# blackfeather-wang/AdaFocus

Measured on AMD Instinct MI355X. Metric: clips/sec (T=16, patch=96^2, ResNet-50 local), higher is better.
Workload: dtype f32; 1 GPU; ActivityNet AdaFocus hot path: gather + ResNet-50 local CNN + GRU classifier, T=16, P=96, B=64 clips/GPU (1024 patches/GPU/step), random-init weights seed 1007; global_batch=64, frames=16, patch=96, parallelism=dp1, streams=3

## Files before the change

adafocus_amd/csrc/adaf_internal.h:

```cpp
#pragma once
#include <hip/hip_runtime.h>
#include <stdint.h>
#include <stddef.h>
#include <string>

#include "../../include/adafocus.h"
#include <type_traits>

struct adaf_handle {
    int device = 0;
    int cus = 256;
    float* zeros = nullptr;
    unsigned* scan_timeouts = nullptr;
    int conv_pos_major = 1;
    int gru_persistent = 1;
    hipEvent_t scan_done[4] = {nullptr, nullptr, nullptr, nullptr};
    bool scan_used[4] = {false, false, false, false};
    int scan_next = 0;
    int scan_resident = 0;
    int scan_slots = 1;
    int bptt_resident = 0;
    std::string err;
};

// ... 78 lines not shown
    }
};

struct AdafOptions {
    int conv_pool = 1;
    int mb_strip = 1;
    int mbv2_chunk = 512;
    int latency_rows = 1536;
    int latency_linear_rows = 128;
    unsigned effnet_plan = 511u;
    unsigned effnet_fused_blocks = 0xffffffffu;
    int effnet_chunk = 1024;
    int stem_rows = 1;
    int split_stage1_f32 = 1;
    int split_lean = 1;
    int tsm_lean = 1;
    int gru_graph_persistent = 0;
    int gru_scan_slices = 2;
};
AdafOptions& adaf_options();

__device__ __forceinline__ _Float16 adaf_f16_of(float v) {
#if defined(__HIP_DEVICE_COMPILE__)
    asm("" : "+v"(v));
#endif
    return (_Float16)v;
}

struct ConvArgs {
    const float* x;
// ... 8 lines not shown
    int ldx, ldo, ldr;
    int act;
    int tsm_T, tsm_fold, tsm_hw;
    const float* zeros;
    int vec_epi;
    int in16, out16, res16;
    int pm_allow;
    int split_n;
    float* out_b;
    int ldo_b, act_b;
    int pm_images, pm_groups;
    int tiles_n;
    int nblocks;
    int pool_hw, pool_rows, pool_ld;
    float* pool_out;
};

int adaf_fail(adaf_handle* h, int code, const char* fmt, ...);
int adaf_hip_fail(adaf_handle* h, hipError_t e, const char* what);
bool adaf_aligned16(const void* p);
enum AdafWsOrder { ADAF_WS_SIZE_FIRST, ADAF_WS_ALIGN_FIRST };
int adaf_check_ws(adaf_handle* h, const char* who, const void* ws, size_t ws_bytes, size_t need, AdafWsOrder order);
int adaf_conv_out(int in, int k, int stride, int pad);
int adaf_make_conv_args(adaf_handle* h, const adaf_conv_params* p, const float* x, const float* w, const float* scale,
                        const float* bias, const float* res, float* out, ConvArgs* a);
int adaf_set_conv_dtypes(adaf_handle* h, bool in16, bool out16, ConvArgs* a);

struct MbFuseArgs {
    const float* x;
    int n, H, W, cin;
// ... 83 lines not shown
                                           float* logits, float* last, int classes, bool cooperative, unsigned* timeouts, hipStream_t s);

int adaf_gru_bptt_blocks_per_cu();
bool adaf_gru_bptt_persistent_ok(int batch, int hidden, int resident_blocks);
hipError_t adaf_launch_gru_bptt(const float* dy, const float* gi, const float* gh, const float* bhh, const float* hs, const float* whh,
                                float* dgi, float* dgh, float* carry, unsigned* bar, unsigned* timeouts, int batch, int steps, int hidden,
                                bool persistent, bool cooperative, hipStream_t s);
void adaf_launch_gemm_strided(const float* A, long long a_m, long long a_k, const float* B, long long b_k, long long b_n, float* C, int ldc,
                              const float* mul, int ldm, int M, int N, int K, hipStream_t s);
size_t adaf_colsum_partial_floats(int cols);
void adaf_launch_colsum(const float* x, int rows, int cols, int ld, float* part, float* out, hipStream_t s);
void adaf_launch_rows_scale(const float* x, const float* mask, float* out, int rows, int width, int steps, bool shift, hipStream_t s);

int adaf_launch_conv_gemm(const ConvArgs& a, int tile, int cus, hipStream_t s);
int adaf_pick_conv_tile(int M, int N, int K, int cus);
int adaf_launch_conv_lat(const ConvArgs& a, hipStream_t s);
int adaf_launch_conv_pool(ConvArgs a, int hw, float* pool_out, int pool_ld, hipStream_t s);
int adaf_launch_conv_pool16(ConvArgs a, int hw, float* pool_out, int pool_ld, hipStream_t s);
int adaf_launch_conv_pool16_rounded(ConvArgs a, int hw, float* pool_out, int pool_ld, hipStream_t s);
bool adaf_conv_tile_exists(int tile);
void adaf_launch_conv_naive(const ConvArgs& a, hipStream_t s);
bool adaf_fused_tail_shift_ok(const ConvArgs& c2, int n3, int ldr, int tsm_T1, int tsm_fold1);
int adaf_launch_fused_tail(const ConvArgs& c2, const float* w3, const float* s3, const float* b3, const float* res, int ldr,
                           float* out, int n3, const float* w1n, const float* s1n, const float* b1n, float* out1, int n1,
                           hipStream_t s, int tsm_T1 = 0, int tsm_fold1 = 0);

hipError_t adaf_launch_crop(const float* frames, int nf, int C, int H, int W, const float* act, int fpa, int P,
                            float* out, int layout, int32_t* coords, hipStream_t s);

hipError_t adaf_launch_crop_resize(const float* frames, int in4, int nf, int C, int H, int W, const float* act, const int32_t* sizes,
// ... 44 lines not shown
```

adafocus_amd/csrc/api.hip:

```cpp
#include <cstdarg>
#include <cstdio>
#include <cstring>

#include "adaf_internal.h"

int adaf_fail(adaf_handle* h, int code, const char* fmt, ...) {
    char buf[512];
    va_list ap;
    va_start(ap, fmt);
    vsnprintf(buf, sizeof(buf), fmt, ap);
    va_end(ap);
    if (h) h->err = buf;
    return code;
}

int adaf_hip_fail(adaf_handle* h, hipError_t e, const char* what) {
    return adaf_fail(h, ADAF_E_LAUNCH, "%s: %s", what, hipGetErrorString(e));
}

bool adaf_aligned16(const void* p) { return (reinterpret_cast<uintptr_t>(p) & 15) == 0; }
int adaf_check_ws(adaf_handle* h, const char* who, const void* ws, size_t ws_bytes, size_t need, AdafWsOrder order) {
    const bool small = ws_bytes < need, skew = !adaf_aligned16(ws);
    if (small && (order == ADAF_WS_SIZE_FIRST || !skew)) return adaf_fail(h, ADAF_E_NOMEM, "%s: workspace %zu < %zu bytes", who, ws_bytes, need);
    return skew ? adaf_fail(h, ADAF_E_LAYOUT, "%s: the workspace must be 16-byte aligned", who) : ADAF_OK;
// ... 15 lines not shown
    if (oh <= 0 || ow <= 0) return adaf_fail(h, ADAF_E_BADARG, "conv: empty output");
    const long long M = (long long)p->n * oh * ow;
    if (M > 0x7fffffffLL || (long long)p->n * p->h * p->w > 0x7fffffffLL) return adaf_fail(h, ADAF_E_BADARG, "conv: too many pixels");
    int fold = 0;
    if (p->tsm_segments > 0) {
        if (p->kh != 1 || p->kw != 1 || p->stride != 1 || p->pad != 0)
            return adaf_fail(h, ADAF_E_BADARG, "conv: fused temporal shift needs a 1x1 stride-1 conv");
        if (p->tsm_div <= 0 || p->n % p->tsm_segments) return adaf_fail(h, ADAF_E_BADARG, "conv: n %% tsm_segments != 0");
        fold = p->cin / p->tsm_div;
        if (fold % 4) return adaf_fail(h, ADAF_E_LAYOUT, "conv: temporal-shift fold=%d must be a multiple of 4", fold);
    }
    a->wsp = nullptr;
    a->in16 = a->out16 = a->res16 = 0;
    a->pm_allow = h->conv_pos_major; a->pm_images = a->pm_groups = 0;
    a->split_n = 0; a->out_b = nullptr; a->ldo_b = 0; a->act_b = 0;
    a->x = x; a->w = w; a->scale = scale; a->bias = bias; a->res = res; a->out = out;
    a->M = (int)M; a->N = p->cout; a->K = p->kh * p->kw * p->cin;
    a->cin = p->cin; a->H = p->h; a->W = p->w; a->OH = oh; a->OW = ow; a->KH = p->kh; a->KW = p->kw;
    a->stride = p->stride; a->pad = p->pad; a->ldx = ldx; a->ldo = ldo; a->ldr = ldr; a->act = p->act;
    a->tsm_T = p->tsm_segments > 0 ? p->tsm_segments : 0; a->tsm_fold = fold; a->tsm_hw = p->h * p->w;
    a->tiles_n = 0; a->nblocks = 0;
    a->zeros = h->zeros;
    a->vec_epi = (p->cout % 4 == 0 && ldo % 4 == 0 && ldr % 4 == 0 && adaf_aligned16(out) && (!res || adaf_aligned16(res)) &&
                  (!scale || adaf_aligned16(scale)) && (!bias || adaf_aligned16(bias))) ? 1 : 0;
    return ADAF_OK;
}

int adaf_set_conv_dtypes(adaf_handle* h, bool in16, bool out16, ConvArgs* a) {
    a->in16 = in16; a->out16 = out16; a->res16 = a->res != nullptr;
    if (in16 && (a->cin % 8 || a->ldx % 8)) return adaf_fail(h, ADAF_E_LAYOUT, "conv_f16: fp16 operands need cin %% 8 == 0 (16-byte chunks)");
    if (in16 && a->tsm_T > 0 && a->tsm_fold % 8)
        return adaf_fail(h, ADAF_E_LAYOUT, "conv_f16: temporal-shift fold=%d must be a multiple of 8 with fp16 operands (whole 16-byte chunks)", a->tsm_fold);
    if (!in16 && a->res) return adaf_fail(h, ADAF_E_BADARG, "conv_f16: a residual needs fp16 operands");
    return ADAF_OK;
}

AdafOptions& adaf_options() {
    static AdafOptions o;
    return o;
}

namespace {
struct OptKey { const char* name; double lo, hi; };
const OptKey kOptKeys[] = {{"conv_pool", 0, 1}, {"mb_strip", 0, 1}, {"mbv2_chunk", 1, 1 << 20}, {"latency_rows", 0, 1 << 30}, {"latency_linear_rows", 0, 1 << 30},
                           {"effnet_plan", 0, 511}, {"effnet_chunk", 1, 1 << 20}, {"gru_scan_slices", 1, 2}, {"effnet_fused_blocks", 0, 4294967295.0},
                           {"stem_rows", 0, 2}, {"split_stage1_f32", 0, 1}, {"gru_graph_persistent", 0, 1}, {"split_lean", 0, 1}, {"tsm_lean", 0, 1}};
int find_opt(const char* key) {
    if (!key) return -1;
    for (size_t i = 0; i < sizeof(kOptKeys) / sizeof(kOptKeys[0]); ++i)
        if (!strcmp(kOptKeys[i].name, key)) return (int)i;
    return -1;
}
}

extern "C" {

int adaf_version(void) { return ADAF_VERSION; }

int adaf_create(int device, adaf_handle** out) {
    if (!out) return ADAF_E_BADARG;
    *out = nullptr;
// ... 50 lines not shown
    AdafOptions& o = adaf_options();
    switch (k) {
        case 0: o.conv_pool = (int)value; break;
        case 1: o.mb_strip = (int)value; break;
        case 2: o.mbv2_chunk = (int)value; break;
        case 3: o.latency_rows = (int)value; break;
        case 4: o.latency_linear_rows = (int)value; break;
        case 5: o.effnet_plan = (unsigned)value; break;
        case 6: o.effnet_chunk = (int)value; break;
        case 7: o.gru_scan_slices = (int)value; break;
        case 8: o.effnet_fused_blocks = (unsigned)value; break;
        case 9: o.stem_rows = (int)value; break;
        case 10: o.split_stage1_f32 = (int)value; break;
        case 11: o.gru_graph_persistent = (int)value; break;
        case 12: o.split_lean = (int)value; break;
        default: o.tsm_lean = (int)value; break;
    }
    return ADAF_OK;
}

double adaf_get_global_option(const char* key) {
    const AdafOptions& o = adaf_options();
    switch (find_opt(key)) {
        case 0: return o.conv_pool;
        case 1: return o.mb_strip;
        case 2: return o.mbv2_chunk;
        case 3: return o.latency_rows;
        case 4: return o.latency_linear_rows;
        case 5: return o.effnet_plan;
        case 6: return o.effnet_chunk;
        case 7: return o.gru_scan_slices;
        case 8: return o.effnet_fused_blocks;
        case 9: return o.stem_rows;
        case 10: return o.split_stage1_f32;
        case 11: return o.gru_graph_persistent;
        case 12: return o.split_lean;
        case 13: return o.tsm_lean;
        default: return __builtin_nan("");
    }
}

int adaf_set_gru_persistent(adaf_handle* h, int on) {
    if (!h) return ADAF_E_BADARG;
    if (on < 0 || on > 2) return adaf_fail(h, ADAF_E_BADARG, "set_gru_persistent: mode %d (0 off, 1 on, 2 on + cooperative launch)", on);
    h->gru_persistent = on;
    return ADAF_OK;
}

int adaf_gru_scan_timeouts(adaf_handle* h, unsigned* count_out) {
    if (!h || !count_out) return ADAF_E_BADARG;
    int cur = 0;
    (void)hipGetDevice(&cur);
// ... 528 lines not shown
```

adafocus_amd/csrc/conv_gemm.hip:

```cpp
#include <cstdlib>
#include <type_traits>
#include <utility>

#include "adaf_internal.h"

typedef float f32x16 __attribute__((ext_vector_type(16)));
typedef float f32x4 __attribute__((ext_vector_type(4)));
typedef float f32x2 __attribute__((ext_vector_type(2)));
typedef unsigned u32x4 __attribute__((ext_vector_type(4)));
typedef __bf16 bf16x8 __attribute__((ext_vector_type(8)));
typedef _Float16 f16x8 __attribute__((ext_vector_type(8)));
typedef _Float16 f16x4 __attribute__((ext_vector_type(4)));

#ifndef CG_ABL
#define CG_ABL 0
#endif

namespace {

typedef __bf16 bf16x2 __attribute__((ext_vector_type(2)));
__device__ __forceinline__ void split3(const f32x4 v0, const f32x4 v1, u32x4& H, u32x4& M, u32x4& L) {
    const float x[8] = {v0.x, v0.y, v0.z, v0.w, v1.x, v1.y, v1.z, v1.w};
    unsigned h[4], m[4], l[4];
#pragma unroll
// ... 440 lines not shown
        }
        if (FLAGS & 1) __builtin_amdgcn_s_setprio(0);
        __builtin_amdgcn_sched_barrier(0);
        if (more) lstore((kt + 1) & 1);
        __syncthreads();
    }

    conv_epilogue<TM, TN, ET>(a, smem, acc, m0, n0, wm, wn, lane, wave);
}


template <int BM, int BN, int WGM, int WGN, bool DENSE, int PIPE, bool SPECIAL, int EMU, bool BSP = false, int DT = 0, bool PM = false,
          bool LEAN = false, bool POOL = false>
__global__ __launch_bounds__(64 * WGM * WGN, (BM == 128 && BN == 128 && WGM * WGN == 4) ? 2 : 1)
void conv_gemm_glds_kernel(const ConvArgs a) {
    static_assert(!POOL || (DENSE && !SPECIAL && ((LEAN && DT == 0) || (!LEAN && (DT == 4 || DT == 6)))),
                  "pooled epilogue: the lean dense fp32 kernel, or the dense fp16-operand kernel with fp32 features (DT 6: fp16 residual, rounded values)");
    static_assert(!PM || (!DENSE && (EMU == 0 || BSP) && PIPE == 1), "position-major tiles: k x k filters on the fp32 pipe, or split tiles with pre-split weights");
    static_assert(!LEAN || ((DENSE || PM) && PIPE == 1 && ((EMU == 0 && !BSP) || (EMU != 0 && BSP)) &&
                            (!SPECIAL || (DENSE && EMU == 0 && DT == 0 && !POOL))),
                  "lean K loop: plain fp32-pipe launches, split tiles with pre-split weights, or (LEAN + SPECIAL) the fp32 pipe's temporally shifted conv1");
    constexpr bool LTSM = LEAN && SPECIAL;
    constexpr int NW = WGM * WGN;
    constexpr int TM = BM / WGM / 32, TN = BN / WGN / 32;
    constexpr int AI = BM / (8 * NW);
    constexpr int BI = BSP ? (3 * BN / 16) / NW : BN / (8 * NW);
    constexpr int STAGE = BM * 32 + BN * (BSP ? 48 : 32);
    static_assert(!BSP || (EMU != 0 && (3 * BN / 16) % NW == 0), "pre-split weights: split tiles only");
    constexpr int SLAB = NW * 32 * (TN * 32 + 4);
    constexpr int POOLF = POOL ? BM * (BN + 4) : 0;
// ... 23 lines not shown
        const int g = tile_m / ohw;
        pm_p = tile_m - g * ohw;
        m0 = g * BM;
        const int oy = pm_p / a.OW, ox = pm_p - oy * a.OW;
        pm_iy0 = oy * a.stride - a.pad;
        pm_ix0 = ox * a.stride - a.pad;
        for (int kh = 0; kh < a.KH; ++kh)
            for (int kw = 0; kw < a.KW; ++kw)
                if ((unsigned)(pm_iy0 + kh) < (unsigned)a.H && (unsigned)(pm_ix0 + kw) < (unsigned)a.W) pm_mask |= 1u << (kh * a.KW + kw);
    }
    const unsigned pm_walk = (PM && a.pm_allow == 2) ? ((1u << (a.KH * a.KW)) - 1u) : pm_mask;

    const int lr = lane >> 3;
    const int ls = lane & 7;
    unsigned va[AI], vb[BI];
    unsigned vnx[LTSM ? AI : 1], vpv[LTSM ? AI : 1];
    const float* lean_a = a.x;
    if (LEAN && PM) lean_a = a.x + ((long long)pm_iy0 * a.W + pm_ix0) * a.ldx;
    const float* pa[AI];
    int step_a[AI];
    long long boff[AI];
    unsigned amask[AI];
    int tflag[AI];
    int qa[AI];
#pragma unroll
    for (int j = 0; j < AI; ++j) {
        const int row = (j * NW + wave) * 8 + lr;
        const int m = m0 + row;
        const bool ok = m < a.M;
        const int mm = ok ? m : 0;
        qa[j] = (ls ^ ((row >> 1) & 7)) * 4;
        pa[j] = a.zeros; step_a[j] = 0; boff[j] = 0; amask[j] = 0; tflag[j] = 0; va[j] = 0;
        if (LEAN) {
            int r = PM ? (m < a.pm_images ? m : 0) : mm;
            if (DENSE && a.stride != 1) {
                const int ohw = a.OH * a.OW;
                const int img = mm / ohw, rem = mm - img * ohw;
                const int oy = rem / a.OW, ox = rem - oy * a.OW;
                r = (img * a.H + oy * a.stride) * a.W + ox * a.stride;
            }
            if constexpr ((CG_ABL & 32) != 0) r &= 1023;
            va[j] = (unsigned)(((size_t)r * (PM ? (size_t)a.H * a.W : (size_t)1) * a.ldx + qa[j]) * 4);
            if constexpr (LTSM) {
                const int t = (mm / a.tsm_hw) % a.tsm_T;
                const unsigned sh = (unsigned)((size_t)a.tsm_hw * a.ldx * 4);
                vnx[j] = (ok && t < a.tsm_T - 1) ? va[j] + sh : 0x7ffffff0u;
                vpv[j] = (ok && t > 0) ? va[j] - sh : 0x7ffffff0u;
            }
        } else if (DENSE) {
            if (ok) { pa[j] = a.x + (size_t)mm * a.ldx + qa[j]; step_a[j] = 32; }
            if (a.tsm_T > 0) {
                const int t = (mm / a.tsm_hw) % a.tsm_T;
                tflag[j] = (ok ? 4 : 0) | (t > 0 ? 1 : 0) | (t < a.tsm_T - 1 ? 2 : 0);
            }
        } else if (PM) {
            const int img = m0 + row;
            const bool iok = img < a.pm_images;
// ... 25 lines not shown
            const int plane = u / (BN / 16), row = (u % (BN / 16)) * 16 + (lane >> 2);
            const int n = n0 + row;
            const int q = ((lane & 3) ^ ((row >> 2) & 3)) * 8;
            qb[j] = q;
            vb[j] = (unsigned)((((size_t)plane * a.N + (n < a.N ? n : 0)) * a.K + q) * 2);
            if (n < a.N) {
                pb[j] = reinterpret_cast<const float*>(a.wsp + ((size_t)plane * a.N + n) * a.K + q);
                step_b[j] = 16;
            } else { pb[j] = a.zeros; step_b[j] = 0; }
        } else {
            const int row = (j * NW + wave) * 8 + lr;
            const int n = n0 + row;
            const int q = (ls ^ ((row >> 1) & 7)) * 4;
            qb[j] = q;
            vb[j] = (unsigned)(((size_t)(n < a.N ? n : 0) * a.K + q) * 4);
            if (n < a.N) { pb[j] = a.w + (size_t)n * a.K + q; step_b[j] = 32; }
            else { pb[j] = a.zeros; step_b[j] = 0; }
        }
    }
    const long long tsm_stride = (long long)a.tsm_hw * a.ldx;

    typedef const __attribute__((address_space(1))) void* gptr_t;
    typedef __attribute__((address_space(3))) void* lptr_t;

    bool nx_tsm = false, nx_tail = false;
    int ltsm_ty = -1;
    unsigned vcur[LTSM ? AI : 1];
    int nx_kt = 0, nx_tap = 0, nx_c0 = 0, nx_kh = 0, nx_kw = 0;
    int nx_koff = 0;
    long long nx_toff = 0;
// ... 77 lines not shown
            src = pa[j];
            if (SPECIAL && nx_tsm) {
                const int c = nx_kt * 32 + qa[j];
                if (c < a.tsm_fold) src = (tflag[j] & 2) ? src + tsm_stride : a.zeros;
                else if (c < 2 * a.tsm_fold) src = (tflag[j] & 1) ? src - tsm_stride : a.zeros;
                if (!(tflag[j] & 4)) src = a.zeros;
            }
            if (SPECIAL && nx_tail && nx_kt * 32 + qa[j] >= a.K) src = a.zeros;
            pa[j] += step_a[j];
        } else {
            src = ((amask[j] >> nx_tap) & 1u) ? a.x + boff[j] + nx_toff : a.zeros;
        }
        __builtin_amdgcn_global_load_lds((gptr_t)src, (lptr_t)(As + j * NW * 8 * 32), 16, 0, 0);
    };
    constexpr int NI = AI + BI;

    f32x16 acc[TM][TN];
#pragma unroll
    for (int i = 0; i < TM; ++i)
#pragma unroll
        for (int j = 0; j < TN; ++j)
#pragma unroll
            for (int r = 0; r < 16; ++r) acc[i][j][r] = 0.f;

    const int sw = (lane >> 1) & 7;
    const int hb = ((lane >> 5) ^ sw) & 1;
    int foff[4];
#pragma unroll
    for (int kk = 0; kk < 4; ++kk) foff[kk] = (lane & 31) * 32 + ((((2 * kk) ^ (sw & 6)) | hb) << 2);
    const int a_base = wm * TM * 32 * 32;
    const int b_base = BM * 32 + wn * TN * 32 * 32;
    int foffe[2][2];
#pragma unroll
    for (int j = 0; j < 2; ++j)
#pragma unroll
        for (int e = 0; e < 2; ++e) foffe[j][e] = (lane & 31) * 32 + (((4 * j + 2 * (lane >> 5) + e) ^ sw) << 2);
    int foffb[2];
#pragma unroll
    for (int j = 0; j < 2; ++j) foffb[j] = (lane & 31) * 16 + ((((2 * j + (lane >> 5)) ^ ((lane >> 2) & 3)) & 3) << 2);

    const int nk = PM ? __builtin_popcount(pm_walk) * (a.cin >> 5) : (a.K + 31) / 32;
    prep(0);
#pragma unroll
    for (int q = 0; q < NI; ++q) issue_one(q, 0);

    if constexpr (EMU != 0 && BSP) {
        constexpr int TA[9] = {2, 2, 1, 2, 0, 1, 1, 0, 0};
        constexpr int TB[9] = {2, 1, 2, 0, 2, 1, 0, 1, 0};
        f32x4 ar[2][TM][2];
        u32x4 bq[2][3][TN];
        auto rd = [&](int sb, const float* St, int j2) {
#pragma unroll
            for (int i = 0; i < TM; ++i) {
                ar[sb][i][0] = *reinterpret_cast<const f32x4*>(St + a_base + i * 1024 + foffe[j2][0]);
                ar[sb][i][1] = *reinterpret_cast<const f32x4*>(St + a_base + i * 1024 + foffe[j2][1]);
            }
#pragma unroll
            for (int j = 0; j < TN; ++j)
#pragma unroll
// ... 128 lines not shown
                __builtin_amdgcn_s_barrier();
                if (has2) prep(k + 2);
                rdf(0, smem + nb1 * STAGE, 0);
            }
            mul(1, has2_tag, 0, QH, k & 1);
        };
        int k = 0;
        for (; k + 2 < nk; ++k) body(k, std::true_type{}, std::true_type{});
        if (nk > 1) { body(k, std::true_type{}, std::false_type{}); ++k; }
        body(k, std::false_type{}, std::false_type{});
        __syncthreads();
        conv_epilogue<TM, TN>(a, smem, acc, m0, n0, wm, wn, lane, wave);
        return;
    }

    auto slice = [&](int kt, auto more_tag, auto stage_tag) {
        constexpr bool more = decltype(more_tag)::value;
        constexpr int stage = decltype(stage_tag)::value;
        asm volatile("s_waitcnt vmcnt(0)" ::: "memory");
        __builtin_amdgcn_s_barrier();
        constexpr int nbuf = stage ^ 1;
        if (more) prep(kt + 1);
        const float* St = smem + stage * STAGE;
        if (!PIPE) {
            if (more) {
#pragma unroll
                for (int q = 0; q < NI; ++q) issue_one(q, nbuf);
            }
        }
        if constexpr (EMU != 0) {
#pragma unroll
            for (int j2 = 0; j2 < 2; ++j2) {
                u32x4 ap[3][TM], bp[3][TN];
// ... 58 lines not shown
                                                                            __builtin_bit_cast(f16x8, bf[cb][j]), acc[i][j], 0, 0, 0);
                if (PIPE) {
                    if (more) {
#pragma unroll
                        for (int q = 0; q < NI; ++q)
                            if ((q * 4) / NI == kk) issue_one(q, nbuf);
                    }
                    __builtin_amdgcn_sched_barrier(0);
                }
            } else {
#pragma unroll
            for (int s4 = 0; s4 < 4; ++s4) {
#pragma unroll
                for (int i = 0; i < TM; ++i)
#pragma unroll
                    for (int j = 0; j < TN; ++j)
                        acc[i][j] = __builtin_amdgcn_mfma_f32_32x32x2f32(af[cb][i][s4], bf[cb][j][s4], acc[i][j], 0, 0, 0);
                if (PIPE && s4 < 2) {
                    if (more) {
#pragma unroll
                        for (int q = 0; q < NI; ++q)
                            if ((q * 8) / NI == 2 * kk + s4) issue_one(q, nbuf);
                    }
                    __builtin_amdgcn_sched_barrier(0);
                }
            }
            }
        }
    };
    {
        using S0 = std::integral_constant<int, 0>;
        using S1 = std::integral_constant<int, 1>;
        int kt = 0;
        for (; kt + 2 < nk; kt += 2) {
            slice(kt, std::true_type{}, S0{});
            slice(kt + 1, std::true_type{}, S1{});
        }
        if (nk - kt == 2) {
            slice(kt, std::true_type{}, S0{});
            slice(kt + 1, std::false_type{}, S1{});
        } else {
            slice(kt, std::false_type{}, S0{});
        }
    }
    __syncthreads();
    if constexpr (POOL) {
        conv_epilogue_pool<TM, TN, BM, BN, NW, DT == 4, DT == 6>(a, smem, acc, m0, n0, wm, wn, lane, wave, tile_m);
        return;
    }
    if (PM) conv_epilogue<TM, TN, (DT & 3)>(a, smem, acc, m0, n0, wm, wn, lane, wave, a.OH * a.OW, pm_p, a.pm_images);
    else conv_epilogue<TM, TN, (DT & 3)>(a, smem, acc, m0, n0, wm, wn, lane, wave);
}

struct FusedTailArgs {
    ConvArgs c2;
    const float* w3;
    const float* s3;
    const float* b3;
    const float* res;
    float* out;
// ... 512 lines not shown
}
constexpr int family_tile(TileFamily fam, int bm, int bn) {
    for (int i = 0; i < kNumTiles; ++i)
        if (kTileTable[i].fam == fam && kTileTable[i].bm == bm && kTileTable[i].bn == bn) return kTileTable[i].id;
    return 0;
}
constexpr int family_tile_like(TileFamily fam, int id) { return family_tile(fam, kTileTable[tile_index(id)].bm, kTileTable[tile_index(id)].bn); }
constexpr int family_pipe(TileFamily f) { return f == TF_BAR23 ? 2 : f == TF_REG || f == TF_DMA_TOP || f == TF_LAT ? 0 : 1; }
constexpr int family_split(TileFamily f) { return f == TF_SPLIT6 || f == TF_PRESPLIT ? 6 : f == TF_SPLIT9 ? 9 : 0; }
constexpr bool has_pos_major_form(const TileRow& r) { return r.fam == TF_DMA_MID || r.fam == TF_PRESPLIT; }
constexpr bool has_lean_form(const TileRow& r) {
    return r.fam == TF_DMA_MID || (r.fam == TF_PRESPLIT && r.bm == 128 && r.bn == 128 && r.wgm == 4 && r.wgn == 1);
}
constexpr bool lean_dense_pays(const TileRow& r) { return has_lean_form(r) && r.bm * r.bn > 64 * 64; }
constexpr bool has_lean_shift_form(const TileRow& r) { return r.fam == TF_DMA_MID && r.bm * r.bn > 64 * 64; }

enum { DT_OUT16 = 1, DT_RES16 = 2, DT_IN16 = 4 };
enum PoolKind { POOL_F32, POOL_F16, POOL_F16_ROUNDED };

struct ConvPlan {
    int tile = -1;
    int row = -1;
    bool dense = false;
    bool gather = false;
    bool special = false;
    bool lean = false;
    bool pos_major = false;
    bool pool = false;
    int dt = 0;
    ConvArgs a;
    explicit ConvPlan(const ConvArgs& conv) : a(conv) {}
};

bool conv_is_dense(const ConvArgs& a) { return a.KH == 1 && a.KW == 1 && a.stride == 1 && a.pad == 0; }
int conv_images(const ConvArgs& a) { return a.OH * a.OW > 0 ? a.M / (a.OH * a.OW) : 0; }

bool dma_reach(size_t elems, size_t elem_bytes = 4) { return elems * elem_bytes < 0xffffff00ull; }
bool operands_in_dma_reach(const ConvArgs& a) {
    return dma_reach((size_t)a.M * a.ldx) && dma_reach((size_t)a.N * a.K) &&
           (conv_is_dense(a) || dma_reach((size_t)a.H * a.W * a.ldx * (size_t)conv_images(a)));
}
bool strided_1x1_as_gather(const ConvArgs& a) {
    return !conv_is_dense(a) && a.KH == 1 && a.KW == 1 && a.pad == 0 && a.stride > 1 && a.tsm_T == 0 && (a.K & 31) == 0;
// ... 54 lines not shown
    }
    for (int i = tile_index(tile); i >= 0; i = tile_index(tile)) {
        const TileRow& r = kTileTable[i];
        if (r.fam == TF_REG || (r.fam == TF_PRESPLIT ? presplit_ok : dma_ok && r.fam != TF_F16 && r.fam != TF_LAT)) return tile;
        tile = r.fallback;
    }
    return -1;
}

void plan_row_major(ConvPlan& p, const ConvArgs& a, int tile, int bm_rows) {
    p.row = tile_index(p.tile = tile);
    p.a.tiles_n = (a.N + kTileTable[p.row].bn - 1) / kTileTable[p.row].bn;
    p.a.nblocks = ((a.M + bm_rows - 1) / bm_rows) * p.a.tiles_n;
}

ConvPlan plan_conv(const ConvArgs& a, int tile, int cus) {
    ConvPlan p(a);
    const bool dense = conv_is_dense(a);
    if (a.in16) {
        if (!conv_glds16_ok(a) || (a.res && !a.res16)) return p;
        if (tile < kTileF16Lo || tile > kTileF16Hi) {
            tile = family_tile_like(TF_F16, adaf_pick_conv_tile(a.M, a.N, a.K, cus));
            if (narrow_output(a) && row_tiles(a, 128) >= cus) tile = family_tile(TF_F16, 128, 32);
        }
        if (tile_index(tile) < 0) return p;
        plan_row_major(p, a, tile, kTileTable[tile_index(tile)].bm);
        p.a.K /= 2; p.a.cin /= 2; p.a.ldx /= 2; p.a.tsm_fold /= 2;
        p.dt = DT_IN16 | DT_RES16 | (a.out16 ? DT_OUT16 : 0);
        p.dense = dense;
        p.special = dense && (a.tsm_T > 0 || (p.a.K & 31));
        return p;
// ... 75 lines not shown
    } else if constexpr (R.fam == TF_F16) {
        constexpr int DT = DT_IN16 | DT_RES16;
        if constexpr (R.id == kTilePoolF16) {
            if (p.pool && (p.dt & DT_RES16)) CONV_GLDS(true, 1, false, 0, false, DT, false, false, true);
            if (p.pool) CONV_GLDS(true, 1, false, 0, false, DT_IN16, false, false, true);
        }
        if (p.special && (p.dt & DT_OUT16)) CONV_GLDS(true, 1, true, 0, false, DT | DT_OUT16);
        if (p.dense && (p.dt & DT_OUT16)) CONV_GLDS(true, 1, false, 0, false, DT | DT_OUT16);
        if (p.dt & DT_OUT16) CONV_GLDS(false, 1, false, 0, false, DT | DT_OUT16);
        if (p.special) CONV_GLDS(true, 1, true, 0, false, DT);
        if (p.dense) CONV_GLDS(true, 1, false, 0, false, DT);
        CONV_GLDS(false, 1, false, 0, false, DT);
    } else {
        constexpr int PIPE = family_pipe(R.fam), EMU = family_split(R.fam);
        constexpr bool BSP = R.fam == TF_PRESPLIT;
        if constexpr (R.id == kTilePoolF32)
            if (p.pool) CONV_GLDS(true, PIPE, false, EMU, BSP, 0, false, true, true);
        if constexpr (has_pos_major_form(R)) {
            if constexpr (has_lean_form(R))
                if (p.pos_major && p.lean) CONV_GLDS(false, PIPE, false, EMU, BSP, 0, true, true);
            if (p.pos_major) CONV_GLDS(false, PIPE, false, EMU, BSP, 0, true);
        }
        if constexpr (has_lean_form(R))
            if (p.lean && !p.special) CONV_GLDS(true, PIPE, false, EMU, BSP, 0, false, true);
        if constexpr (has_lean_shift_form(R))
            if (p.lean && p.special) CONV_GLDS(true, PIPE, true, EMU, BSP, 0, false, true);
        if (p.special) CONV_GLDS(true, PIPE, true, EMU, BSP);
        if (p.dense) CONV_GLDS(true, PIPE, false, EMU, BSP);
        CONV_GLDS(false, PIPE, false, EMU, BSP);
    }
// ... 26 lines not shown
    (void)K;
    int best = 1;
    double best_t = 1e300;
    for (const TileRow& r : kTileTable) {
        if (r.eff <= 0.f) continue;
        const long long blocks = (long long)((M + r.bm - 1) / r.bm) * ((N + r.bn - 1) / r.bn);
        const long long rounds = (blocks + cus - 1) / cus;
        const double cost = (double)rounds * r.bm * r.bn / r.eff;
        if (cost < best_t * 0.999) { best_t = cost; best = r.id; }
    }
    return best;
}

bool adaf_conv_tile_exists(int tile) { return tile == kTileAutoSplit || tile_index(tile) >= 0; }

int adaf_launch_conv_gemm(const ConvArgs& a, int tile, int cus, hipStream_t s) { return launch_plan(plan_conv(a, tile, cus), s); }

int adaf_launch_conv_pool(ConvArgs a, int hw, float* pool_out, int pool_ld, hipStream_t s) {
    return launch_conv_pool(a, hw, pool_out, pool_ld, POOL_F32, s);
}

int adaf_launch_conv_pool16(ConvArgs a, int hw, float* pool_out, int pool_ld, hipStream_t s) {
    return launch_conv_pool(a, hw, pool_out, pool_ld, POOL_F16, s);
}

int adaf_launch_conv_pool16_rounded(ConvArgs a, int hw, float* pool_out, int pool_ld, hipStream_t s) {
    return launch_conv_pool(a, hw, pool_out, pool_ld, POOL_F16_ROUNDED, s);
}

extern "C" int adaf_conv_plan_debug(const adaf_conv_params* p, int flags, int cus, int* out, int n) {
    enum { IN16 = 1, OUT16 = 2, RES16 = 4, PRESPLIT = 8, VEC_EPI = 64 };
    alignas(16) static const float operand[4] = {0.f, 0.f, 0.f, 0.f};
    alignas(16) static float result[4];
    if (!out || cus <= 0) return ADAF_E_BADARG;
    adaf_handle host;
    ConvArgs a;
    int rc = adaf_make_conv_args(&host, p, operand, operand, nullptr, nullptr, (flags & RES16) ? operand : nullptr, result, &a);
    if (!rc && (flags & (IN16 | OUT16 | RES16))) rc = adaf_set_conv_dtypes(&host, (flags & IN16) != 0, (flags & OUT16) != 0, &a);
    if (rc) return rc;
    if (flags & PRESPLIT) a.wsp = reinterpret_cast<const unsigned short*>(operand);
    a.pm_allow = (flags >> 4) & 3;
    a.vec_epi = a.vec_epi && (flags & VEC_EPI);
    const int hw = flags >> 8;
    const ConvPlan c = hw > 0 ? plan_conv_pool(a, hw, operand, p->cout, !a.in16 ? POOL_F32 : a.res16 ? POOL_F16_ROUNDED : POOL_F16)
                              : plan_conv(a, p->tile, cus);
    const TileRow r = c.row >= 0 ? kTileTable[c.row] : TileRow{0, 0, 0, 0, 0, TF_REG, 0, 0, 0.f};
    const int kPlanFields[] = {c.tile, r.bm, r.bn, r.wgm, r.wgn, (int)r.fam, r.fallback, family_pipe(r.fam), family_split(r.fam),
                               r.fam == TF_PRESPLIT, c.dt, c.dense, c.gather, c.special, c.lean, c.pos_major, c.pool, c.a.tiles_n, c.a.nblocks,
                               c.a.pm_images, c.a.pm_groups, c.a.vec_epi, c.a.K, c.a.cin, c.a.ldx, c.a.tsm_fold};
    for (int i = 0; i < n && i < (int)(sizeof(kPlanFields) / sizeof(int)); ++i) out[i] = kPlanFields[i];
    return ADAF_OK;
}

void adaf_launch_conv_naive(const ConvArgs& a, hipStream_t s) {
    const long long total = (long long)a.M * a.N;
    hipLaunchKernelGGL(conv_naive_kernel, dim3((unsigned)((total + 255) / 256)), dim3(256), 0, s, a);
}

static bool fused_tail_pm(const ConvArgs& c2, int n3, int ldr, int* images_out, int* groups_out, int gstride = 128) {
    const int ohw = c2.OH * c2.OW;
    const int images = ohw > 0 ? c2.M / ohw : 0;
    const int groups = (images + gstride - 1) / gstride;
    *images_out = images;
    *groups_out = groups;
    return c2.pm_allow == 1 && images * ohw == c2.M && images >= 128 && ohw <= 4096 &&
           (long long)groups * 128 * 100 <= (long long)images * (gstride == 128 ? 106 : 108) && (size_t)ohw * 8 * (size_t)(n3 > ldr ? n3 : ldr) * 4 < 0xffffff00ull;
// ... 51 lines not shown
```

adafocus_amd/csrc/resnet_trunk.hip:

```cpp
#include <cstdio>
#include <cstring>
#include <string>
#include <vector>

#include "adaf_net.h"

struct ConvLayer : AdafNetConv {
    int pad;
    bool tsm = false;
    unsigned short* wsp = nullptr;
};

struct adaf_resnet50 {
    adaf_handle* h = nullptr;
    AdafParamTable params;
    AdafWeightArena arena;
    std::vector<ConvLayer> convs;
    std::vector<int> tiles;
    int blocks[4] = {3, 4, 6, 3};
    float* l10_w = nullptr;
    float* l10_scale = nullptr;
    float* l10_bias = nullptr;
    unsigned short* l10_w16 = nullptr;
    int math = ADAF_MATH_F32;
// ... 214 lines not shown
                am.split_n = C1.cout;
                am.out_b = f16 ? reinterpret_cast<float*>(reinterpret_cast<_Float16*>(dsb) - C1.cout) : dsb - C1.cout;
                am.ldo_b = DS.cout;
                am.act_b = ADAF_ACT_NONE;
                const double M = (double)am.M;
                mark(2.0 * M * (C1.cout + DS.cout) * C1.cin, eb * (M * C1.cin + M * (C1.cout + DS.cout) + (double)(C1.cout + DS.cout) * C1.cin), 93);
                if (adaf_launch_conv_gemm(am, f16 ? 82 : 32, h->cus, st) < 0) return adaf_fail(h, ADAF_E_LAUNCH, "resnet50%s: merged layer1.0 launch", tag);
                h1 = am.OH; w1 = am.OW;
                ++li;
                ds_done = true;
            } else if (!c1_done) {
                if ((rc = conv(cur, hh, ww, ADAF_ACT_RELU, nullptr, t1, tsm_c1 > 0 && net->convs[li].tsm, &h1, &w1))) return rc;
            } else ++li;
            c1_done = false;
            const float* identity = cur;
            if (b == 0) {
                if (!ds_done) {
                    li = i_ds;
                    int hd, wd;
                    if ((rc = conv(cur, hh, ww, ADAF_ACT_NONE, nullptr, dsb, false, &hd, &wd))) return rc;
                }
                identity = dsb;
            }
            li = i_c2;
            const ConvLayer& L2 = net->convs[i_c2];
            const bool fusable = fuse && stage1_f32 && L2.cin == 64 && L2.cout == 64 && L2.stride == 1 &&
                                 !net->tiles[i_c2] && !net->tiles[i_c3] && (net->fuse_stem_always || (long long)n * h1 * w1 * 2 >= 3ll * 128 * h->cus);
            if (fusable) {
                const ConvLayer& L3 = net->convs[i_c3];
                const adaf_conv_params p = layer_params(L2, n, h1, w1, ADAF_ACT_RELU);
                ConvArgs a2;
                if ((rc = adaf_make_conv_args(h, &p, t1, L2.w, L2.scale, L2.bias, nullptr, t2, &a2))) return rc;
// ... 14 lines not shown
            } else {
                if ((rc = conv(t1, h1, w1, ADAF_ACT_RELU, nullptr, t2, false, &h2, &w2))) return rc;
                const bool last = s == 3 && b == net->blocks[3] - 1;
                if (last && fuse && !rec && !featmap && net->math != ADAF_MATH_F32_SPLIT_BF16 && !net->tiles[li] && !(lat_ok && n * h2 * w2 <= lat_rows)) {
                    const ConvLayer& L3 = net->convs[li];
                    const adaf_conv_params p = layer_params(L3, n, h2, w2, ADAF_ACT_RELU);
                    ConvArgs a3;
                    if ((rc = adaf_make_conv_args(h, &p, t2, bank(L3), L3.scale, L3.bias, identity, nxt, &a3))) return rc;
                    if (f16) a3.in16 = a3.res16 = 1;
                    if (f16 ? adaf_launch_conv_pool16_rounded(a3, h2 * w2, feat, ldfeat, st) : adaf_launch_conv_pool(a3, h2 * w2, feat, ldfeat, st)) {
                        pooled = true;
                        h3 = h2; w3 = w2;
                        ++li;
                    }
                }
                if (!pooled && (rc = conv(t2, h2, w2, ADAF_ACT_RELU, identity, nxt, false, &h3, &w3))) return rc;
            }
            li = i_next;
            hh = h3; ww = w3;
            float* t = cur; cur = nxt; nxt = t;
        }
    }
    if (featmap) {
        if (f16) adaf_launch_cast(cur, (long long)n * hh * ww * 2048, featmap, 0, st);
        else (void)hipMemcpyAsync(featmap, cur, (size_t)n * hh * ww * 2048 * sizeof(float), hipMemcpyDeviceToDevice, st);
    }
    if (!pooled) {
        mark(0.0, eb * (double)n * hh * ww * 2048 + 4.0 * (double)n * 2048, 0);
        if (f16) adaf_launch_avgpool_f16(cur, n, hh * ww, 2048, feat, ldfeat, st);
        else adaf_launch_avgpool(cur, n, hh * ww, 2048, feat, ldfeat, st);
    }
// ... 255 lines not shown
```

Measured before the change: 5531 clips/s.

## Fuse downsample 1x1 conv into conv3 GEMM with dual accumulator chains

Adds a DUAL variant of the lean dense fp32 GEMM kernel that runs the downsample 1x1 conv's K loop into a second accumulator, then conv3's K loop, and combines both in the epilogue with their BN scale and bias plus ReLU. In stages 2-4 the first bottleneck block now issues one kernel instead of a separate downsample conv and conv3 with a residual read. This removes the dsb intermediate's write and re-read and one launch. In exchange the kernel holds double accumulators, which raises register pressure and may lower occupancy. It is gated by a new ds_in_conv3 option that defaults to on.

Measured after the change: 5557 clips/s (median of 6 runs). Within noise of the previous version (+0.5%).

```diff
diff --git a/adafocus_amd/csrc/adaf_internal.h b/adafocus_amd/csrc/adaf_internal.h
--- a/adafocus_amd/csrc/adaf_internal.h
+++ b/adafocus_amd/csrc/adaf_internal.h
@@ -116,6 +116,7 @@
     int stem_rows = 1;
     int split_stage1_f32 = 1;
     int split_lean = 1;
+    int ds_in_conv3 = 1;
     int tsm_lean = 1;
     int gru_graph_persistent = 0;
     int gru_scan_slices = 2;
@@ -154,6 +155,11 @@
     int nblocks;
     int pool_hw, pool_rows, pool_ld;
     float* pool_out;
+    const float* x2;
+    const float* w2;
+    const float* scale2;
+    const float* bias2;
+    int K2, ldx2, H2, W2, stride2;
 };
 
 int adaf_fail(adaf_handle* h, int code, const char* fmt, ...);
@@ -267,6 +273,8 @@
 
 int adaf_launch_conv_gemm(const ConvArgs& a, int tile, int cus, hipStream_t s);
 int adaf_pick_conv_tile(int M, int N, int K, int cus);
+bool adaf_conv_add_branch(ConvArgs* a, const ConvArgs& branch);
+bool adaf_conv_dual_ok(const ConvArgs& a, int tile, int cus);
 int adaf_launch_conv_lat(const ConvArgs& a, hipStream_t s);
 int adaf_launch_conv_pool(ConvArgs a, int hw, float* pool_out, int pool_ld, hipStream_t s);
 int adaf_launch_conv_pool16(ConvArgs a, int hw, float* pool_out, int pool_ld, hipStream_t s);
diff --git a/adafocus_amd/csrc/api.hip b/adafocus_amd/csrc/api.hip
--- a/adafocus_amd/csrc/api.hip
+++ b/adafocus_amd/csrc/api.hip
@@ -53,6 +53,7 @@
     a->in16 = a->out16 = a->res16 = 0;
     a->pm_allow = h->conv_pos_major; a->pm_images = a->pm_groups = 0;
     a->split_n = 0; a->out_b = nullptr; a->ldo_b = 0; a->act_b = 0;
+    a->x2 = a->w2 = a->scale2 = a->bias2 = nullptr; a->K2 = a->ldx2 = a->H2 = a->W2 = a->stride2 = 0;
     a->x = x; a->w = w; a->scale = scale; a->bias = bias; a->res = res; a->out = out;
     a->M = (int)M; a->N = p->cout; a->K = p->kh * p->kw * p->cin;
     a->cin = p->cin; a->H = p->h; a->W = p->w; a->OH = oh; a->OW = ow; a->KH = p->kh; a->KW = p->kw;
@@ -83,7 +84,7 @@
 struct OptKey { const char* name; double lo, hi; };
 const OptKey kOptKeys[] = {{"conv_pool", 0, 1}, {"mb_strip", 0, 1}, {"mbv2_chunk", 1, 1 << 20}, {"latency_rows", 0, 1 << 30}, {"latency_linear_rows", 0, 1 << 30},
                            {"effnet_plan", 0, 511}, {"effnet_chunk", 1, 1 << 20}, {"gru_scan_slices", 1, 2}, {"effnet_fused_blocks", 0, 4294967295.0},
-                           {"stem_rows", 0, 2}, {"split_stage1_f32", 0, 1}, {"gru_graph_persistent", 0, 1}, {"split_lean", 0, 1}, {"tsm_lean", 0, 1}};
+                           {"stem_rows", 0, 2}, {"split_stage1_f32", 0, 1}, {"gru_graph_persistent", 0, 1}, {"split_lean", 0, 1}, {"tsm_lean", 0, 1}, {"ds_in_conv3", 0, 1}};
 int find_opt(const char* key) {
     if (!key) return -1;
     for (size_t i = 0; i < sizeof(kOptKeys) / sizeof(kOptKeys[0]); ++i)
@@ -164,7 +165,8 @@
         case 10: o.split_stage1_f32 = (int)value; break;
         case 11: o.gru_graph_persistent = (int)value; break;
         case 12: o.split_lean = (int)value; break;
-        default: o.tsm_lean = (int)value; break;
+        case 13: o.tsm_lean = (int)value; break;
+        default: o.ds_in_conv3 = (int)value; break;
     }
     return ADAF_OK;
 }
@@ -186,6 +188,7 @@
         case 11: return o.gru_graph_persistent;
         case 12: return o.split_lean;
         case 13: return o.tsm_lean;
+        case 14: return o.ds_in_conv3;
         default: return __builtin_nan("");
     }
 }
diff --git a/adafocus_amd/csrc/conv_gemm.hip b/adafocus_amd/csrc/conv_gemm.hip
--- a/adafocus_amd/csrc/conv_gemm.hip
+++ b/adafocus_amd/csrc/conv_gemm.hip
@@ -478,6 +478,9 @@
           bool LEAN = false, bool POOL = false>
 __global__ __launch_bounds__(64 * WGM * WGN, (BM == 128 && BN == 128 && WGM * WGN == 4) ? 2 : 1)
 void conv_gemm_glds_kernel(const ConvArgs a) {
+    constexpr bool DUAL = (DT & 8) != 0;
+    static_assert(!DUAL || (DT == 8 && LEAN && DENSE && !SPECIAL && EMU == 0 && !BSP && PIPE == 1 && !PM && !POOL),
+                  "two accumulator chains: the lean dense fp32 kernel with the DMA between the MFMA groups");
     static_assert(!POOL || (DENSE && !SPECIAL && ((LEAN && DT == 0) || (!LEAN && (DT == 4 || DT == 6)))),
                   "pooled epilogue: the lean dense fp32 kernel, or the dense fp16-operand kernel with fp32 features (DT 6: fp16 residual, rounded values)");
     static_assert(!PM || (!DENSE && (EMU == 0 || BSP) && PIPE == 1), "position-major tiles: k x k filters on the fp32 pipe, or split tiles with pre-split weights");
@@ -531,6 +534,7 @@
     const int lr = lane >> 3;
     const int ls = lane & 7;
     unsigned va[AI], vb[BI];
+    unsigned va2[DUAL ? AI : 1], vb2[DUAL ? BI : 1];
     unsigned vnx[LTSM ? AI : 1], vpv[LTSM ? AI : 1];
     const float* lean_a = a.x;
     if (LEAN && PM) lean_a = a.x + ((long long)pm_iy0 * a.W + pm_ix0) * a.ldx;
@@ -558,6 +562,13 @@
             }
             if constexpr ((CG_ABL & 32) != 0) r &= 1023;
             va[j] = (unsigned)(((size_t)r * (PM ? (size_t)a.H * a.W : (size_t)1) * a.ldx + qa[j]) * 4);
+            if constexpr (DUAL) {
+                const int ohw = a.OH * a.OW;
+                const int img = mm / ohw, rem = mm - img * ohw;
+                const int oy = rem / a.OW, ox = rem - oy * a.OW;
+                const size_t r2 = ((size_t)img * a.H2 + oy * a.stride2) * a.W2 + ox * a.stride2;
+                va2[j] = (unsigned)((r2 * a.ldx2 + qa[j]) * 4);
+            }
             if constexpr (LTSM) {
                 const int t = (mm / a.tsm_hw) % a.tsm_T;
                 const unsigned sh = (unsigned)((size_t)a.tsm_hw * a.ldx * 4);
@@ -613,6 +624,7 @@
             const int q = (ls ^ ((row >> 1) & 7)) * 4;
             qb[j] = q;
             vb[j] = (unsigned)(((size_t)(n < a.N ? n : 0) * a.K + q) * 4);
+            if constexpr (DUAL) vb2[j] = (unsigned)(((size_t)(n < a.N ? n : 0) * a.K2 + q) * 4);
             if (n < a.N) { pb[j] = a.w + (size_t)n * a.K + q; step_b[j] = 32; }
             else { pb[j] = a.zeros; step_b[j] = 0; }
         }
@@ -720,6 +732,11 @@
         __builtin_amdgcn_global_load_lds((gptr_t)src, (lptr_t)(As + j * NW * 8 * 32), 16, 0, 0);
     };
     constexpr int NI = AI + BI;
+    auto issue_dual = [&](int q, int buf, auto d_tag) {
+        constexpr bool D = decltype(d_tag)::value;
+        if (q < BI) lean_dma((D ? a.w2 : a.w) + nx_kt * 32, D ? vb2[q] : vb[q], smem + buf * STAGE + BM * 32 + (wave + q * NW) * 8 * 32);
+        else lean_dma((D ? a.x2 : a.x) + nx_kt * 32, D ? va2[q - BI] : va[q - BI], smem + buf * STAGE + (wave + (q - BI) * NW) * 8 * 32);
+    };
 
     f32x16 acc[TM][TN];
 #pragma unroll
@@ -728,6 +745,15 @@
         for (int j = 0; j < TN; ++j)
 #pragma unroll
             for (int r = 0; r < 16; ++r) acc[i][j][r] = 0.f;
+    f32x16 acc2[DUAL ? TM : 1][DUAL ? TN : 1];
+    if constexpr (DUAL) {
+#pragma unroll
+        for (int i = 0; i < TM; ++i)
+#pragma unroll
+            for (int j = 0; j < TN; ++j)
+#pragma unroll
+                for (int r = 0; r < 16; ++r) acc2[i][j][r] = 0.f;
+    }
 
     const int sw = (lane >> 1) & 7;
     const int hb = ((lane >> 5) ^ sw) & 1;
@@ -748,7 +774,10 @@
     const int nk = PM ? __builtin_popcount(pm_walk) * (a.cin >> 5) : (a.K + 31) / 32;
     prep(0);
 #pragma unroll
-    for (int q = 0; q < NI; ++q) issue_one(q, 0);
+    for (int q = 0; q < NI; ++q) {
+        if constexpr (DUAL) issue_dual(q, 0, std::true_type{});
+        else issue_one(q, 0);
+    }
 
     if constexpr (EMU != 0 && BSP) {
         constexpr int TA[9] = {2, 2, 1, 2, 0, 1, 1, 0, 0};
@@ -907,9 +936,10 @@
         return;
     }
 
-    auto slice = [&](int kt, auto more_tag, auto stage_tag) {
+    auto slice = [&](int kt, auto more_tag, auto stage_tag, auto accd_tag, auto nxd_tag) {
         constexpr bool more = decltype(more_tag)::value;
         constexpr int stage = decltype(stage_tag)::value;
+        constexpr bool accd = DUAL && decltype(accd_tag)::value;
         asm volatile("s_waitcnt vmcnt(0)" ::: "memory");
         __builtin_amdgcn_s_barrier();
         constexpr int nbuf = stage ^ 1;
@@ -998,13 +1028,18 @@
 #pragma unroll
                 for (int i = 0; i < TM; ++i)
 #pragma unroll
-                    for (int j = 0; j < TN; ++j)
-                        acc[i][j] = __builtin_amdgcn_mfma_f32_32x32x2f32(af[cb][i][s4], bf[cb][j][s4], acc[i][j], 0, 0, 0);
+                    for (int j = 0; j < TN; ++j) {
+                        if constexpr (accd) acc2[i][j] = __builtin_amdgcn_mfma_f32_32x32x2f32(af[cb][i][s4], bf[cb][j][s4], acc2[i][j], 0, 0, 0);
+                        else acc[i][j] = __builtin_amdgcn_mfma_f32_32x32x2f32(af[cb][i][s4], bf[cb][j][s4], acc[i][j], 0, 0, 0);
+                    }
                 if (PIPE && s4 < 2) {
                     if (more) {
 #pragma unroll
                         for (int q = 0; q < NI; ++q)
-                            if ((q * 8) / NI == 2 * kk + s4) issue_one(q, nbuf);
+                            if ((q * 8) / NI == 2 * kk + s4) {
+                                if constexpr (DUAL) issue_dual(q, nbuf, nxd_tag);
+                                else issue_one(q, nbuf);
+                            }
                     }
                     __builtin_amdgcn_sched_barrier(0);
                 }
@@ -1015,19 +1050,54 @@
     {
         using S0 = std::integral_constant<int, 0>;
         using S1 = std::integral_constant<int, 1>;
+        using T = std::true_type;
+        using F = std::false_type;
+        if constexpr (DUAL) {
+            const int nkd = a.K2 >> 5;
+            int kd = 0;
+            for (; kd + 2 < nkd; kd += 2) {
+                slice(kd, T{}, S0{}, T{}, T{});
+                slice(kd + 1, T{}, S1{}, T{}, T{});
+            }
+            slice(kd, T{}, S0{}, T{}, T{});
+            slice(-1, T{}, S1{}, T{}, F{});
+        }
         int kt = 0;
         for (; kt + 2 < nk; kt += 2) {
-            slice(kt, std::true_type{}, S0{});
-            slice(kt + 1, std::true_type{}, S1{});
+            slice(kt, T{}, S0{}, F{}, F{});
+            slice(kt + 1, T{}, S1{}, F{}, F{});
         }
         if (nk - kt == 2) {
-            slice(kt, std::true_type{}, S0{});
-            slice(kt + 1, std::false_type{}, S1{});
+            slice(kt, T{}, S0{}, F{}, F{});
+            slice(kt + 1, F{}, S1{}, F{}, F{});
         } else {
-            slice(kt, std::false_type{}, S0{});
+            slice(kt, F{}, S0{}, F{}, F{});
         }
     }
     __syncthreads();
+    if constexpr (DUAL) {
+        const float act_lo = a.act == ADAF_ACT_NONE ? -__builtin_inff() : 0.f;
+        const float act_hi = a.act == ADAF_ACT_RELU6 ? 6.f : __builtin_inff();
+#pragma unroll
+        for (int j = 0; j < TN; ++j) {
+            const int n = n0 + (wn * TN + j) * 32 + (lane & 31);
+            const int nn = n < a.N ? n : 0;
+            const float sc = a.scale ? a.scale[nn] : 1.f, bi = a.bias ? a.bias[nn] : 0.f;
+            const float sc2 = a.scale2 ? a.scale2[nn] : 1.f, bi2 = a.bias2 ? a.bias2[nn] : 0.f;
+#pragma unroll
+            for (int i = 0; i < TM; ++i)
+#pragma unroll
+                for (int r = 0; r < 16; ++r) {
+                    const float id = __builtin_fmaf(acc2[i][j][r], sc2, bi2);
+                    acc[i][j][r] = __builtin_amdgcn_fmed3f(__builtin_fmaf(acc[i][j][r], sc, bi) + id, act_lo, act_hi);
+                }
+        }
+        ConvArgs o = a;
+        o.scale = o.bias = o.res = nullptr;
+        o.act = ADAF_ACT_NONE;
+        conv_epilogue<TM, TN>(o, smem, acc, m0, n0, wm, wn, lane, wave);
+        return;
+    }
     if constexpr (POOL) {
         conv_epilogue_pool<TM, TN, BM, BN, NW, DT == 4, DT == 6>(a, smem, acc, m0, n0, wm, wn, lane, wave, tile_m);
         return;
@@ -1570,8 +1640,9 @@
 }
 constexpr bool lean_dense_pays(const TileRow& r) { return has_lean_form(r) && r.bm * r.bn > 64 * 64; }
 constexpr bool has_lean_shift_form(const TileRow& r) { return r.fam == TF_DMA_MID && r.bm * r.bn > 64 * 64; }
-
-enum { DT_OUT16 = 1, DT_RES16 = 2, DT_IN16 = 4 };
+constexpr bool has_dual_form(const TileRow& r) { return r.fam == TF_DMA_MID && r.bn == 64 && r.wgm == 2 && r.wgn == 2 && (r.bm == 128 || r.bm == 64); }
+
+enum { DT_OUT16 = 1, DT_RES16 = 2, DT_IN16 = 4, DT_DUAL = 8 };
 enum PoolKind { POOL_F32, POOL_F16, POOL_F16_ROUNDED };
 
 struct ConvPlan {
@@ -1583,6 +1654,7 @@
     bool lean = false;
     bool pos_major = false;
     bool pool = false;
+    bool dual = false;
     int dt = 0;
     ConvArgs a;
     explicit ConvPlan(const ConvArgs& conv) : a(conv) {}
@@ -1667,7 +1739,23 @@
     p.a.nblocks = ((a.M + bm_rows - 1) / bm_rows) * p.a.tiles_n;
 }
 
+ConvPlan plan_conv_dual(const ConvArgs& a, int tile, int cus) {
+    ConvPlan p(a);
+    if (!adaf_options().ds_in_conv3 || !conv_is_dense(a) || a.in16 || a.out16 || a.res16 || a.res || a.wsp || a.split_n || a.tsm_T > 0) return p;
+    if ((a.K & 31) || (a.K2 & 63) || a.K2 <= 0 || a.stride2 <= 0 || !operands_in_dma_reach(a) || !dma_reach((size_t)a.N * a.K2) ||
+        !dma_reach((size_t)conv_images(a) * a.H2 * a.W2 * a.ldx2))
+        return p;
+    if (tile <= 0) tile = family_tile(TF_DMA_MID, kTileTable[tile_index(adaf_pick_conv_tile(a.M, a.N, a.K, cus))].bm, 64);
+    if (tile_index(tile) < 0 || !has_dual_form(kTileTable[tile_index(tile)])) return p;
+    plan_row_major(p, a, tile, kTileTable[tile_index(tile)].bm);
+    if (a.vec_epi) p.a.vec_epi = 2;
+    p.dense = p.lean = p.dual = true;
+    p.dt = DT_DUAL;
+    return p;
+}
+
 ConvPlan plan_conv(const ConvArgs& a, int tile, int cus) {
+    if (a.x2) return plan_conv_dual(a, tile, cus);
     ConvPlan p(a);
     const bool dense = conv_is_dense(a);
     if (a.in16) {
@@ -1773,6 +1861,9 @@
     } else {
         constexpr int PIPE = family_pipe(R.fam), EMU = family_split(R.fam);
         constexpr bool BSP = R.fam == TF_PRESPLIT;
+        if constexpr (has_dual_form(R))
+            if (p.dual) CONV_GLDS(true, PIPE, false, EMU, BSP, DT_DUAL, false, true);
+        if (p.dual) return -1;
         if constexpr (R.id == kTilePoolF32)
             if (p.pool) CONV_GLDS(true, PIPE, false, EMU, BSP, 0, false, true, true);
         if constexpr (has_pos_major_form(R)) {
@@ -1829,6 +1920,17 @@
 
 bool adaf_conv_tile_exists(int tile) { return tile == kTileAutoSplit || tile_index(tile) >= 0; }
 
+bool adaf_conv_add_branch(ConvArgs* a, const ConvArgs& b) {
+    const bool relu_like = a->act == ADAF_ACT_NONE || a->act == ADAF_ACT_RELU || a->act == ADAF_ACT_RELU6;
+    if (!conv_is_dense(*a) || a->res || !relu_like || b.KH != 1 || b.KW != 1 || b.pad != 0 || b.tsm_T > 0 || b.res || b.act != ADAF_ACT_NONE ||
+        b.in16 || b.out16 || a->in16 || a->out16 || b.M != a->M || b.N != a->N || b.OH != a->OH || b.OW != a->OW)
+        return false;
+    a->x2 = b.x; a->w2 = b.w; a->scale2 = b.scale; a->bias2 = b.bias;
+    a->K2 = b.K; a->ldx2 = b.ldx; a->H2 = b.H; a->W2 = b.W; a->stride2 = b.stride;
+    return true;
+}
+bool adaf_conv_dual_ok(const ConvArgs& a, int tile, int cus) { return a.x2 != nullptr && plan_conv_dual(a, tile, cus).tile > 0; }
+
 int adaf_launch_conv_gemm(const ConvArgs& a, int tile, int cus, hipStream_t s) { return launch_plan(plan_conv(a, tile, cus), s); }
 
 int adaf_launch_conv_pool(ConvArgs a, int hw, float* pool_out, int pool_ld, hipStream_t s) {
@@ -1843,7 +1945,7 @@
     return launch_conv_pool(a, hw, pool_out, pool_ld, POOL_F16_ROUNDED, s);
 }
 
-extern "C" int adaf_conv_plan_debug(const adaf_conv_params* p, int flags, int cus, int* out, int n) {
+static int conv_plan_debug(const adaf_conv_params* p, const adaf_conv_params* branch, int flags, int cus, int* out, int n) {
     enum { IN16 = 1, OUT16 = 2, RES16 = 4, PRESPLIT = 8, VEC_EPI = 64 };
     alignas(16) static const float operand[4] = {0.f, 0.f, 0.f, 0.f};
     alignas(16) static float result[4];
@@ -1852,6 +1954,13 @@
     ConvArgs a;
     int rc = adaf_make_conv_args(&host, p, operand, operand, nullptr, nullptr, (flags & RES16) ? operand : nullptr, result, &a);
     if (!rc && (flags & (IN16 | OUT16 | RES16))) rc = adaf_set_conv_dtypes(&host, (flags & IN16) != 0, (flags & OUT16) != 0, &a);
+    if (!rc && branch) {
+        ConvArgs b, pair = a;
+        rc = adaf_make_conv_args(&host, branch, operand, operand, nullptr, nullptr, nullptr, result, &b);
+        if (!rc && !adaf_conv_add_branch(&pair, b)) rc = ADAF_E_BADARG;
+        pair.vec_epi = pair.vec_epi && (flags & VEC_EPI);
+        if (!rc && adaf_conv_dual_ok(pair, p->tile, cus)) a = pair;
+    }
     if (rc) return rc;
     if (flags & PRESPLIT) a.wsp = reinterpret_cast<const unsigned short*>(operand);
     a.pm_allow = (flags >> 4) & 3;
@@ -1865,6 +1974,25 @@
                                c.a.pm_images, c.a.pm_groups, c.a.vec_epi, c.a.K, c.a.cin, c.a.ldx, c.a.tsm_fold};
     for (int i = 0; i < n && i < (int)(sizeof(kPlanFields) / sizeof(int)); ++i) out[i] = kPlanFields[i];
     return ADAF_OK;
+}
+extern "C" int adaf_conv_plan_debug(const adaf_conv_params* p, int flags, int cus, int* out, int n) { return conv_plan_debug(p, nullptr, flags, cus, out, n); }
+extern "C" int adaf_conv_dual_plan_debug(const adaf_conv_params* p, const adaf_conv_params* branch, int flags, int cus, int* out, int n) {
+    return branch ? conv_plan_debug(p, branch, flags, cus, out, n) : ADAF_E_BADARG;
+}
+
+extern "C" int adaf_conv_dual_debug(adaf_handle* h, const adaf_conv_params* p, const float* x, const float* w, const float* scale, const float* bias,
+                                    const adaf_conv_params* branch, const float* x2, const float* w2, const float* scale2, const float* bias2,
+                                    float* out, void* stream) {
+    if (!h) return ADAF_E_BADARG;
+    ConvArgs a, b;
+    int rc = adaf_make_conv_args(h, p, x, w, scale, bias, nullptr, out, &a);
+    if (!rc) rc = adaf_make_conv_args(h, branch, x2, w2, scale2, bias2, nullptr, out, &b);
+    if (rc) return rc;
+    if (!adaf_conv_add_branch(&a, b)) return adaf_fail(h, ADAF_E_BADARG, "conv_dual: the branch is not a 1x1 conv over the same output pixels and channels");
+    if (!adaf_conv_dual_ok(a, p->tile, h->cus)) return adaf_fail(h, ADAF_E_BADARG, "conv_dual: no dual launch for this pair (tile %d, K %d + %d)", p->tile, a.K, a.K2);
+    if (adaf_launch_conv_gemm(a, p->tile, h->cus, (hipStream_t)stream) < 0) return adaf_fail(h, ADAF_E_LAUNCH, "conv_dual: no tile");
+    hipError_t e = hipGetLastError();
+    return e == hipSuccess ? ADAF_OK : adaf_hip_fail(h, e, "conv_dual launch");
 }
 
 void adaf_launch_conv_naive(const ConvArgs& a, hipStream_t s) {
diff --git a/adafocus_amd/csrc/resnet_trunk.hip b/adafocus_amd/csrc/resnet_trunk.hip
--- a/adafocus_amd/csrc/resnet_trunk.hip
+++ b/adafocus_amd/csrc/resnet_trunk.hip
@@ -252,8 +252,20 @@
             } else ++li;
             c1_done = false;
             const float* identity = cur;
+            bool ds_in_c3 = false;
+            ConvArgs a3d;
+            if (s > 0 && b == 0 && fuse && net->math == ADAF_MATH_F32 && !net->tiles[i_c3] && !net->tiles[i_ds]) {
+                const ConvLayer &C2 = net->convs[i_c2], &C3 = net->convs[i_c3], &DS = net->convs[i_ds];
+                const adaf_conv_params p3 = layer_params(C3, n, adaf_conv_out(h1, C2.k, C2.stride, C2.pad), adaf_conv_out(w1, C2.k, C2.stride, C2.pad), ADAF_ACT_RELU);
+                const adaf_conv_params pd = layer_params(DS, n, hh, ww, ADAF_ACT_NONE);
+                ConvArgs ad;
+                if ((rc = adaf_make_conv_args(h, &p3, t2, C3.w, C3.scale, C3.bias, nullptr, nxt, &a3d)) ||
+                    (rc = adaf_make_conv_args(h, &pd, cur, DS.w, DS.scale, DS.bias, nullptr, dsb, &ad)))
+                    return rc;
+                ds_in_c3 = !(lat_ok && a3d.M <= lat_rows) && adaf_conv_add_branch(&a3d, ad) && adaf_conv_dual_ok(a3d, 0, h->cus);
+            }
             if (b == 0) {
-                if (!ds_done) {
+                if (!ds_done && !ds_in_c3) {
                     li = i_ds;
                     int hd, wd;
                     if ((rc = conv(cur, hh, ww, ADAF_ACT_NONE, nullptr, dsb, false, &hd, &wd))) return rc;
@@ -298,7 +310,15 @@
                         ++li;
                     }
                 }
-                if (!pooled && (rc = conv(t2, h2, w2, ADAF_ACT_RELU, identity, nxt, false, &h3, &w3))) return rc;
+                if (ds_in_c3) {
+                    const ConvLayer &C3 = net->convs[li], &DS = net->convs[i_ds];
+                    const double M = (double)a3d.M;
+                    mark(2.0 * M * C3.cout * (C3.cin + DS.cin),
+                         4.0 * ((double)n * hh * ww * DS.cin + M * C3.cin + M * C3.cout + (double)C3.cout * (C3.cin + DS.cin)), 97);
+                    if (adaf_launch_conv_gemm(a3d, 0, h->cus, st) < 0) return adaf_fail(h, ADAF_E_LAUNCH, "resnet50: conv3 + downsample launch (conv launch %d)", li);
+                    h3 = a3d.OH; w3 = a3d.OW;
+                    ++li;
+                } else if (!pooled && (rc = conv(t2, h2, w2, ADAF_ACT_RELU, identity, nxt, false, &h3, &w3))) return rc;
             }
             li = i_next;
             hh = h3; ww = w3;
```
